# nyu-systems/Grendel-GS

Hardware: NVIDIA B200
Metric: train-step Gaussians/s (preprocess+forward+loss+backward) (higher is better)
Workload: dtype f32

## Files before the change

### grendel-gs_b200/csrc/blend.cu

```cuda
#include "common.cuh"

#define BL_THREADS 256
#define BL_WARPS (BL_THREADS / 32)
#define BL_BLOCKS 16
#ifndef FW_CHUNK
#define FW_CHUNK 256
#endif

#define ALPHA_MIN (1.0f / 255.0f)
#define ALPHA_MAX 0.99f
#define T_EPS 0.0001f
#define FULL 0xffffffffu

GS_D float gs_exp_neg(float x) {
    float y;
    asm("ex2.approx.ftz.f32 %0, %1;" : "=f"(y) : "f"(x * 1.4426950408889634f));
    return y;
}

struct Where { int blk, px, py, half, l16; };
GS_D Where where_am_i(int tile, int gx) {
    Where p;
    const int w = threadIdx.x >> 5, lane = threadIdx.x & 31;
    p.half = lane >> 4;
// ... 174 lines not shown
                        const float test_T = T * (1.f - alpha);
                        if (test_T < T_EPS) {
                            done = true;
                            pxf = qnan;
                            if (STATS) considered = (uint32_t)(base + j + 1);
                        } else {
                            const float2 gb = *reinterpret_cast<const float2 *>(&sr->c);
                            const float w = alpha * T;
                            C0 += b.w * w; C1 += gb.x * w; C2 += gb.y * w;
                            T = test_T;
                            last = (uint32_t)(base + j + 1);
                            if (STATS) blended++;
                        }
                    }
                }
            }
        }
    }
    if (inside) {
        image[pix] = (Ct0 + C0) + T * bg[0];
        image[HW + pix] = (Ct1 + C1) + T * bg[1];
        image[2 * HW + pix] = (Ct2 + C2) + T * bg[2];
        final_T[pix] = T;
        n_contrib[pix] = last;
        if (considered == 0) considered = (uint32_t)total;
    }
    if (CKPT) {
        float r0 = C0, r1 = C1, r2 = C2;
        for (int s = nck - 1; s >= 0; s--) {
            const float4 c = ck[(size_t)s * SEG_SLOT];
            ck[(size_t)s * SEG_SLOT] = make_float4(c.x, r0, r1, r2);
            r0 += c.y; r1 += c.z; r2 += c.w;
        }
        uint32_t m = inside ? last : 0u;
#pragma unroll
        for (int o = 16; o > 0; o >>= 1) m = max(m, __shfl_xor_sync(FULL, m, o));
        if (lane == 0) s_red[threadIdx.x >> 5] = m;
        __syncthreads();
        if (threadIdx.x == 0) {
            uint32_t tl = 0;
#pragma unroll
            for (int w = 0; w < BL_WARPS; w++) tl = max(tl, s_red[w]);
            const uint32_t nseg = (tl + SEG_K - 1) / SEG_K;
            seg.tile_last[blockIdx.x] = tl;
            s_red[BL_WARPS] = nseg;
            s_red[BL_WARPS + 1] = nseg ? atomicAdd(seg.n_units, nseg) : 0u;
        }
        __syncthreads();
        const uint32_t nseg = s_red[BL_WARPS], ubase = s_red[BL_WARPS + 1];
        for (uint32_t i = threadIdx.x; i < nseg; i += BL_THREADS) seg.units[ubase + i] = make_uint2(blockIdx.x, nseg - 1 - i);
    }
    if (STATS) {
        if (threadIdx.x < 3) s_stats[threadIdx.x] = 0ull;
        __syncthreads();
        unsigned long long v0 = inside ? (unsigned long long)total : 0ull, v1 = inside ? considered : 0u,
                           v2 = inside ? blended : 0u;
#pragma unroll
        for (int o = 16; o > 0; o >>= 1) {
            v0 += __shfl_xor_sync(FULL, v0, o);
            v1 += __shfl_xor_sync(FULL, v1, o);
            v2 += __shfl_xor_sync(FULL, v2, o);
        }
        if (lane == 0) { atomicAdd(&s_stats[0], v0); atomicAdd(&s_stats[1], v1); atomicAdd(&s_stats[2], v2); }
        __syncthreads();
        if (threadIdx.x < 3) atomicAdd(&stats[3 * view + threadIdx.x], s_stats[threadIdx.x]);
    }
}

#define F2_THREADS 128
#define F2_WARPS 4
#ifndef F2_MIN_CTAS
#define F2_MIN_CTAS 8
#endif
typedef unsigned long long p2;
GS_D p2 p2_make(float lo, float hi) { p2 r; asm("mov.b64 %0, {%1, %2};" : "=l"(r) : "f"(lo), "f"(hi)); return r; }
GS_D p2 p2_bc(float v) { return p2_make(v, v); }
GS_D float p2_lo(p2 v) { float lo, hi; asm("mov.b64 {%0, %1}, %2;" : "=f"(lo), "=f"(hi) : "l"(v)); return lo; }
GS_D float p2_hi(p2 v) { float lo, hi; asm("mov.b64 {%0, %1}, %2;" : "=f"(lo), "=f"(hi) : "l"(v)); return hi; }
GS_D p2 p2_fma(p2 a, p2 b, p2 c) { p2 r; asm("fma.rn.f32x2 %0, %1, %2, %3;" : "=l"(r) : "l"(a), "l"(b), "l"(c)); return r; }
GS_D p2 p2_mul(p2 a, p2 b) { p2 r; asm("mul.rn.f32x2 %0, %1, %2;" : "=l"(r) : "l"(a), "l"(b)); return r; }
GS_D p2 p2_add(p2 a, p2 b) { p2 r; asm("add.rn.f32x2 %0, %1, %2;" : "=l"(r) : "l"(a), "l"(b)); return r; }
GS_D void p2_fma_acc(p2 &c, p2 a, p2 b) { asm("fma.rn.f32x2 %0, %1, %2, %0;" : "+l"(c) : "l"(a), "l"(b)); }
GS_D void p2_mul_acc(p2 &t, p2 f) { asm("mul.rn.f32x2 %0, %0, %1;" : "+l"(t) : "l"(f)); }

template <bool STATS, bool CKPT>
__global__ void __launch_bounds__(F2_THREADS, F2_MIN_CTAS)
k_blend_fwd2(int W, int H, int tiles_per_view, const float4 *__restrict__ rec, const float *__restrict__ bg,
             const uint8_t *__restrict__ compute_locally, const uint2 *__restrict__ ranges,
             const uint32_t *__restrict__ ids, float *__restrict__ image, float *__restrict__ final_T,
             uint32_t *__restrict__ n_contrib, unsigned long long *__restrict__ stats, const SegWs seg) {
    __shared__ SRec s_rec[FW_CHUNK + 1];
    __shared__ uint16_t s_cull[FW_CHUNK];
    __shared__ unsigned long long s_stats[3];
    __shared__ uint32_t s_red[F2_WARPS + 2];
    const int gx = (W + GS_BLOCK_X - 1) / GS_BLOCK_X;
    const int view = blockIdx.x / tiles_per_view, tile = blockIdx.x - view * tiles_per_view;
    const int warp = threadIdx.x >> 5, lane = threadIdx.x & 31;
    const int quarter = lane >> 3, l8 = lane & 7;
    const int lx = quarter * 4 + (l8 & 1) * 2, ly = warp * 4 + (l8 >> 1);
    const int px = (tile % gx) * GS_BLOCK_X + lx, py = (tile / gx) * GS_BLOCK_Y + ly;
    const bool in0 = px < W && py < H, in1 = px + 1 < W && py < H;
    const size_t HW = (size_t)H * W;
    const size_t pix = (size_t)py * W + px;
    image += (size_t)view * 3 * HW;
    final_T += (size_t)view * HW;
    n_contrib += (size_t)view * HW;
    if (!compute_locally[blockIdx.x]) {
        if (in0) { image[pix] = 0.f; image[HW + pix] = 0.f; image[2 * HW + pix] = 0.f; }
        if (in1) { image[pix + 1] = 0.f; image[HW + pix + 1] = 0.f; image[2 * HW + pix + 1] = 0.f; }
        if (CKPT && threadIdx.x == 0) seg.tile_last[blockIdx.x] = 0u;
        return;
    }
    const uint2 range = ranges[blockIdx.x];
    const int total = (int)(range.y - range.x);
    const float X0 = (float)((tile % gx) * GS_BLOCK_X), Y0 = (float)((tile / gx) * GS_BLOCK_Y);
    const float qnan = __int_as_float(0x7fc00000);
    float npx0 = in0 ? -(float)px : qnan, npx1 = in1 ? -(float)(px + 1) : qnan;
    const float pyf = (float)py;
    const p2 zero2 = p2_bc(0.f), one2 = p2_bc(1.f), mone2 = p2_bc(-1.f);
    p2 T = one2, C0 = zero2, C1 = zero2, C2 = zero2, Ct0 = zero2, Ct1 = zero2, Ct2 = zero2;
    uint32_t last0 = 0, last1 = 0, blended = 0, cons0 = 0, cons1 = 0;
#define F2_DONE (npx0 != npx0 && npx1 != npx1)
    float4 *ck = nullptr;
    int nck = 0;
    if (CKPT)
        ck = seg.ckpt + ((size_t)(range.x / SEG_K) + blockIdx.x) * SEG_SLOT + (warp * 2 + (lx >> 3)) * 32 + (ly & 3) * 8 + (lx & 7);
    for (int i = threadIdx.x; i < FW_CHUNK + 1; i += F2_THREADS) {
        const float4 z = make_float4(0.f, 0.f, 0.f, 0.f);
        s_rec[i].a = z; s_rec[i].b = z; s_rec[i].c = z;
    }
    for (int base = 0; base < total; base += FW_CHUNK) {
        if (__syncthreads_count(F2_DONE) == F2_THREADS) break;
        const int cnt = min(FW_CHUNK, total - base);
        for (int i = threadIdx.x; i < cnt; i += F2_THREADS) {
            const uint32_t g = ids[range.x + base + i];
            const float4 *r = rec + (size_t)3 * g;
            const float4 a = __ldg(r), b = __ldg(r + 1), c = __ldg(r + 2);
            s_rec[i].a = make_float4(a.x, a.y, -a.z, -a.w);
            s_rec[i].b = make_float4(-b.x, b.y, fmaxf(-b.z, 0.f), b.w);
            s_rec[i].c = c;
            const uint16_t m16 = (uint16_t)block_mask16(a, b, c.z, c.w, X0, Y0);
            s_cull[i] = m16;
            if (CKPT) seg.cull[range.x + base + i] = m16;
        }
        __syncthreads();
        for (int g0 = 0; g0 < cnt; g0 += 32) {
            if (__all_sync(FULL, F2_DONE)) break;
            {
                const int e0 = base + g0;
                if (e0 > 0 && (e0 & (SEG_K - 1)) == 0) {
                    if (CKPT) {
                        ck[(size_t)nck * SEG_SLOT] = make_float4(p2_lo(T), p2_lo(C0), p2_lo(C1), p2_lo(C2));
                        ck[(size_t)nck * SEG_SLOT + 1] = make_float4(p2_hi(T), p2_hi(C0), p2_hi(C1), p2_hi(C2));
                        nck++;
                    }
                    Ct0 = p2_add(Ct0, C0); Ct1 = p2_add(Ct1, C1); Ct2 = p2_add(Ct2, C2);
                    C0 = C1 = C2 = zero2;
                }
            }
            const int jj = g0 + 31 - lane;
            const uint32_t m = jj < cnt ? ((uint32_t)s_cull[jj] >> (warp * 4)) : 0u;
            const uint32_t c0 = __ballot_sync(FULL, m & 1u), c1 = __ballot_sync(FULL, m & 2u),
                           c2 = __ballot_sync(FULL, m & 4u), c3 = __ballot_sync(FULL, m & 8u);
            uint32_t mine = quarter == 0 ? c0 : quarter == 1 ? c1 : quarter == 2 ? c2 : c3;
            const p2 npx = p2_make(npx0, npx1);
            p2 npx_cur = npx;
// ... 366 lines not shown
    const uint4 *s_role = &s_role_all[warp][lane];
    const SegCold *s_cold = &s_cold_all[warp];
    const float pxf0 = (float)(X0 + (lane & 7)), pyf0 = (float)(Y0 + (lane >> 3));
    for (int pass = (cnt - 1) / SG_STAGE; pass >= 0; pass--) {
        const int p0 = pass * SG_STAGE;
        __syncwarp();
        const SegCold cold = *s_cold;
        const int pn = min(SG_STAGE, cold.cnt - p0);
        if (lane < pn) {
            const int i = p0 + lane;
            const uint32_t g = cold.ids[i];
            const float4 *r = rec + (size_t)3 * g;
            const float4 a = __ldg(r), b = __ldg(r + 1), c = __ldg(r + 2);
            uint32_t m = cold.cull[i];
            m = (m | (m >> 1)) & 0x5555u;
            m = (m | (m >> 1)) & 0x3333u;
            m = (m | (m >> 2)) & 0x0f0fu;
            m = (m | (m >> 4)) & 0x00ffu;
#pragma unroll
            for (int q = 0; q < 8; q++) {
                const uint32_t bl = ((q < 4 ? cold.blive : cold.blive_hi) >> (8 * (q & 3))) & 0xffu;
                if ((uint32_t)i >= bl) m &= ~(1u << q);
            }
            s_rec[lane].a = make_float4(a.x, a.y, -a.z, -a.w);
            s_rec[lane].b = make_float4(-b.x, b.y, fmaxf(-b.z, 0.f), b.w);
            s_rec[lane].c = make_float4(c.x, c.y, gs_rcp_approx(b.y), __uint_as_float(g));
            s_mask[lane] = m;
        }
        __syncwarp();
        for (int jl = pn - 1; jl >= 0; jl--) {
            const uint32_t m8 = __reduce_or_sync(FULL, s_mask[jl]);
            if (m8 == 0u) continue;
            const int j = p0 + jl;
            const float4 a = s_rec[jl].a, b4 = s_rec[jl].b;
            const float2 c4 = *reinterpret_cast<const float2 *>(&s_rec[jl].c);
            const float mxl = a.x - pxf0, myl = a.y - pyf0;
            float v[9];
#pragma unroll
            for (int q = 0; q < 9; q++) v[q] = 0.f;
            bool any_full = false;
#pragma unroll
            for (int b = 0; b < 8; b++) {
                if (m8 & (1u << b)) {
                    const float4 pc = s_pix[b * 32];
                    const float dx = mxl - (float)((b & 1) * 8), dy = myl - (float)((b >> 1) * 4);
                    const float q = dx * (a.z * dx + a.w * dy) + b4.x * dy * dy;
                    const bool ok = (j < __float_as_int(pc.w)) && __float_as_uint(q) <= __float_as_uint(b4.z);
                    if (__any_sync(FULL, ok)) {
                        const float G = gs_exp_neg(-q);
                        const float alpha = fminf(ALPHA_MAX, b4.y * G);
                        const float ae = ok ? alpha : 0.f;
                        float inv;
                        asm("rcp.approx.ftz.f32 %0, %1;" : "=f"(inv) : "f"(1.f - ae));
                        const float Tk = T[b] * inv;
                        T[b] = Tk;
                        const float cd = b4.w * pc.x + c4.x * pc.y + c4.y * pc.z;
                        const float dL_dalpha = cd * Tk - S[b] * inv;
                        const float mw = ok ? b4.y * dL_dalpha * G : 0.f;
                        const float dch = ae * Tk;
                        S[b] += dch * cd;
                        const float mx_ = mw * dx, my_ = mw * dy;
                        v[0] += mx_; v[1] += my_; v[2] += mx_ * dx; v[3] += mx_ * dy; v[4] += my_ * dy; v[5] += mw;
                        v[6] += dch * pc.x; v[7] += dch * pc.y; v[8] += dch * pc.z;
                        any_full = true;
                    }
                }
            }
            if (!any_full) continue;
            {
                const float sx = v[0], sy = v[1];
                v[0] = 2.f * a.z * sx + a.w * sy;
                v[1] = 2.f * b4.x * sy + a.w * sx;
                v[5] *= s_rec[jl].c.z;
            }
            warp_reduce9(v, lane);
            const uint4 ro = *s_role;
            const float val = (lane == 1 ? v[8] : v[0]) * __uint_as_float(ro.w);
            float *rptr = reinterpret_cast<float *>((unsigned long long)ro.x | ((unsigned long long)ro.y << 32));
            if (rptr) asm volatile("red.global.add.f32 [%0], %1;" ::"l"(rptr + (size_t)__float_as_uint(s_rec[jl].c.w) * ro.z), "f"(val) : "memory");
        }
    }
}

template <bool STATS, bool CKPT>
static void launch_fwd(int grid, cudaStream_t stream, int W, int H, int T1, const float *rec, const float *bg,
                       const uint8_t *cl, const uint32_t *ranges, const uint32_t *ids, float *image, float *final_T,
                       uint32_t *n_contrib, int64_t *stats, const SegWs &seg) {
    if (g_gs_debug_flags & GS_DEBUG_FWD_HALFWARP)
        k_blend_fwd<STATS, CKPT><<<grid, BL_THREADS, 0, stream>>>(
            W, H, T1, reinterpret_cast<const float4 *>(rec), bg, cl, reinterpret_cast<const uint2 *>(ranges), ids, image,
            final_T, n_contrib, reinterpret_cast<unsigned long long *>(stats), seg);
    else
        k_blend_fwd2<STATS, CKPT><<<grid, F2_THREADS, 0, stream>>>(
            W, H, T1, reinterpret_cast<const float4 *>(rec), bg, cl, reinterpret_cast<const uint2 *>(ranges), ids, image,
            final_T, n_contrib, reinterpret_cast<unsigned long long *>(stats), seg);
}

int gs_launch_blend_forward(int num_views, int64_t R, int H, int W, const float *rec, const float *bg,
                            const uint8_t *compute_locally, const uint32_t *ranges, const uint32_t *ids_sorted,
                            float *image, float *final_T, uint32_t *n_contrib, int64_t *stats, void *seg_ws,
                            size_t seg_ws_bytes, cudaStream_t stream) {
    const int gx = (W + GS_BLOCK_X - 1) / GS_BLOCK_X, gy = (H + GS_BLOCK_Y - 1) / GS_BLOCK_Y;
    const int T1 = gx * gy;
    SegWs seg = {nullptr, nullptr, nullptr, nullptr};
    if (seg_ws) {
        if (seg_ws_bytes < seg_bytes(R, (int64_t)T1 * num_views)) {
            gs_set_error("gs_render_forward: segment workspace too small (%zu < %zu)", seg_ws_bytes,
                         seg_bytes(R, (int64_t)T1 * num_views));
            return GS_ENOMEM;
        }
        GS_REQUIRE(((uintptr_t)seg_ws & 255) == 0, "segment workspace must be 256-byte aligned");
        seg = seg_carve(seg_ws, R, (int64_t)T1 * num_views);
        GS_CUDA_TRY(cudaMemsetAsync(seg.n_units, 0, 256, stream));
    }
    if (stats) GS_CUDA_TRY(cudaMemsetAsync(stats, 0, 3 * sizeof(int64_t) * (size_t)num_views, stream));
    GsStageTimer timer(GS_STAGE_BLEND_FWD, stream);
    const int grid = T1 * num_views;
    if (stats && seg_ws)
        launch_fwd<true, true>(grid, stream, W, H, T1, rec, bg, compute_locally, ranges, ids_sorted, image, final_T, n_contrib, stats, seg);
    else if (stats)
        launch_fwd<true, false>(grid, stream, W, H, T1, rec, bg, compute_locally, ranges, ids_sorted, image, final_T, n_contrib, stats, seg);
    else if (seg_ws)
        launch_fwd<false, true>(grid, stream, W, H, T1, rec, bg, compute_locally, ranges, ids_sorted, image, final_T, n_contrib, stats, seg);
    else
        launch_fwd<false, false>(grid, stream, W, H, T1, rec, bg, compute_locally, ranges, ids_sorted, image, final_T, n_contrib, stats, seg);
    GS_LAUNCH_CHECK();
    return GS_OK;
}

extern "C" int gs_render_backward(int P, int64_t R, int image_height, int image_width, const float *rec,
                                  const float *bg, const uint8_t *compute_locally, const uint32_t *ranges,
                                  const uint32_t *ids_sorted, const float *final_T, const uint32_t *n_contrib,
                                  const float *dL_dimage, const void *seg_ws, size_t seg_ws_bytes, float *dL_dmeans2D,
                                  float *dL_dconic_opacity, float *dL_drgb, void *stream) {
    return gs_render_backward_batched(1, P, R, image_height, image_width, rec, bg, compute_locally, ranges, ids_sorted,
                                      final_T, n_contrib, dL_dimage, seg_ws, seg_ws_bytes, dL_dmeans2D, dL_dconic_opacity,
                                      dL_drgb, stream);
}

extern "C" int gs_render_backward_batched(int num_views, int P, int64_t R, int image_height, int image_width,
                                          const float *rec, const float *bg, const uint8_t *compute_locally,
                                          const uint32_t *ranges, const uint32_t *ids_sorted, const float *final_T,
                                          const uint32_t *n_contrib, const float *dL_dimage, const void *seg_ws,
                                          size_t seg_ws_bytes, float *dL_dmeans2D, float *dL_dconic_opacity,
                                          float *dL_drgb, void *stream_) {
    cudaStream_t stream = (cudaStream_t)stream_;
    GS_REQUIRE(num_views >= 1 && num_views <= GS_MAX_VIEWS, "num_views must be in [1, GS_MAX_VIEWS]");
    GS_REQUIRE(P >= 0 && R >= 0 && image_height > 0 && image_width > 0, "sizes");
    if (P == 0) return GS_OK;
    GS_REQUIRE(dL_dmeans2D && dL_dconic_opacity && dL_drgb, "null output");
    if (dL_dmeans2D == dL_dconic_opacity + 4 * (size_t)P && dL_drgb == dL_dmeans2D + 2 * (size_t)P) {
        GS_CUDA_TRY(cudaMemsetAsync(dL_dconic_opacity, 0, sizeof(float) * 9 * (size_t)P, stream));
    } else {
        GS_CUDA_TRY(cudaMemsetAsync(dL_dmeans2D, 0, sizeof(float) * 2 * (size_t)P, stream));
        GS_CUDA_TRY(cudaMemsetAsync(dL_dconic_opacity, 0, sizeof(float) * 4 * (size_t)P, stream));
        GS_CUDA_TRY(cudaMemsetAsync(dL_drgb, 0, sizeof(float) * 3 * (size_t)P, stream));
    }
    if (R == 0) return GS_OK;
    GS_REQUIRE(rec && bg && compute_locally && ranges && ids_sorted && final_T && n_contrib && dL_dimage, "null input");
    const int gx = (image_width + GS_BLOCK_X - 1) / GS_BLOCK_X, gy = (image_height + GS_BLOCK_Y - 1) / GS_BLOCK_Y;
    GsStageTimer timer(GS_STAGE_BLEND_BWD, stream);
    if (seg_ws && !(g_gs_debug_flags & GS_DEBUG_BWD_TILE)) {
        const int64_t T = (int64_t)gx * gy * num_views;
        if (seg_ws_bytes < seg_bytes(R, T)) {
            gs_set_error("gs_render_backward: segment workspace too small");
            return GS_ENOMEM;
        }
        const SegWs seg = seg_carve(const_cast<void *>(seg_ws), R, T);
        const int64_t max_units = R / SEG_K + T;
        k_blend_bwd_seg<<<(unsigned)((max_units + SG_WARPS - 1) / SG_WARPS), SG_THREADS, 0, stream>>>(
            image_width, image_height, gx * gy, reinterpret_cast<const float4 *>(rec), bg,
            reinterpret_cast<const uint2 *>(ranges), ids_sorted, final_T, n_contrib, dL_dimage, seg, dL_dmeans2D,
            dL_dconic_opacity, dL_drgb);
        GS_LAUNCH_CHECK();
        return GS_OK;
    }
    k_blend_bwd<<<gx * gy * num_views, BL_THREADS, 0, stream>>>(
        image_width, image_height, gx * gy, reinterpret_cast<const float4 *>(rec), bg, compute_locally,
        reinterpret_cast<const uint2 *>(ranges), ids_sorted, final_T, n_contrib, dL_dimage, dL_dmeans2D, dL_dconic_opacity,
        dL_drgb);
    GS_LAUNCH_CHECK();
    return GS_OK;
}
```

### grendel-gs_b200/gs_b200/_lib.py

```python
import ctypes as C
import os

_PKG = os.path.dirname(os.path.dirname(os.path.abspath(__file__)))
LIB_PATH = os.environ.get("GS_B200_LIB") or os.path.join(_PKG, "lib", "libgrendel_gs_b200.so")

_vp, _i, _f, _i64, _sz = C.c_void_p, C.c_int, C.c_float, C.c_int64, C.c_size_t

SIGNATURES = {
    "gs_last_error": (C.c_char_p, []),
    "gs_version": (C.c_char_p, []),
    "gs_get_block_xy": (_i, [C.POINTER(_i)] * 3),
    "gs_preprocess_forward": (_i, [_i, _i, _vp, _vp, _f, _vp, _vp, _vp, _vp, _vp, _vp, _i, _i, _f, _f,
                                   _vp, _vp, _vp, _vp, _vp, _vp, _vp]),
    "gs_preprocess_backward": (_i, [_i, _i, _vp, _vp, _f, _vp, _vp, _vp, _vp, _vp, _i, _i, _f, _f, _vp, _vp,
                                    _vp, _vp, _vp, _vp, _vp, _vp, _vp, _vp, _vp]),
    "gs_preprocess_forward_raw": (_i, [_i, _i, _vp, _vp, _vp, _vp, _f, _vp, _vp, _vp, _vp, _vp, _i, _i, _f, _f,
                                       _vp, _vp, _vp, _vp, _vp, _vp, _vp]),
    "gs_preprocess_backward_raw": (_i, [_i, _i, _vp, _vp, _vp, _vp, _f, _vp, _vp, _vp, _vp, _vp, _i, _i, _f, _f,
                                        _vp, _vp, _vp, _vp, _vp, _vp, _vp, _vp, _vp, _vp, _vp, _vp]),
    "gs_preprocess_forward_batched": (_i, [_i, _i, _i, _vp, _vp, _vp, _vp, _f, _vp, _vp, _vp, _i, _i,
                                           _vp, _vp, _vp, _vp, _vp, _vp, _vp]),
    "gs_preprocess_backward_batched": (_i, [_i, _i, _i, _vp, _vp, _vp, _vp, _f, _vp, _vp, _vp, _i, _i, _vp, _vp,
                                            _vp, _vp, _vp, _vp, _vp, _vp, _vp, _vp, _vp, _vp]),
    "gs_get_local2j_ids_bool": (_i, [_i, _i, _i, _i, _vp, _vp, _vp, _vp, _vp]),
# ... 22 lines not shown
    "gs_profile_stage_name": (C.c_char_p, [_i]),
    "gs_debug_set": (_i, [_i]),
    "gs_loss_temp_bytes": (_sz, [_i, _i]),
    "gs_loss_forward": (_i, [_i, _i, _i, _i, _i, _i, _vp, _vp, _vp, _vp, _sz, _vp]),
    "gs_loss_backward": (_i, [_i, _i, _i, _i, _i, _i, _vp, _vp, _vp, _vp, _vp, _vp, _vp]),
    "gs_route_scan_temp_bytes": (_sz, [_i, _i]),
    "gs_route_scan": (_i, [_i, _i, _vp, _vp, _vp, _vp, _sz, _vp]),
    "gs_xchg_temp_bytes": (_sz, [_i, _i, _i]),
    "gs_xchg_route": (_i, [_i, _i, _i, _i, _i, _vp, _vp, _vp, _vp, _vp, _vp, _vp, _vp, _sz, _vp]),
    "gs_xchg_pack": (_i, [_i, _i, _i, _vp, _vp, _vp, _vp, _vp, _vp, _vp, _vp, _vp]),
    "gs_xchg_unpack": (_i, [_i, _vp, _vp, _vp, _vp, _i, _vp, _i, _vp, _vp, _vp, _vp, _vp, _vp]),
    "gs_xchg_pack_grad": (_i, [_i, _vp, _vp, _vp, _vp, _i, _i, _vp, _vp, _vp, _vp, _vp]),
    "gs_xchg_scatter_grad": (_i, [_i, _i, _i, _vp, _vp, _vp, _vp, _vp, _vp, _vp]),
    "gs_adam_step": (_i, [_i, _vp, _vp, _vp, _vp, _vp, _vp, _vp, _vp, _vp, _vp, C.c_float, _vp]),
    "gs_knn3_mean_dist2": (_i, [_i, _vp, _vp, _vp]),
    "gs_densify_temp_bytes": (_sz, [_i]),
    "gs_densify_select": (_i, [_i, _vp, _vp, _vp, _vp, C.c_float, C.c_float, C.c_float, C.c_float, _i, _vp, _sz, _vp, _vp]),
    "gs_densify_gather": (_i, [_i, _i, _i, _i, _vp, _vp, _vp, _vp, _vp, _vp, _vp, _vp, _vp]),
    "gs_peer_alloc": (_i, [_sz, C.POINTER(C.c_void_p), _vp]),
    "gs_peer_open": (_i, [_vp, C.POINTER(C.c_void_p)]),
    "gs_peer_close": (_i, [_vp]),
    "gs_peer_free": (_i, [_vp]),
    "gs_xchg_pack_p2p": (_i, [_i, _i, _i, _vp, _vp, _vp, _vp, _vp, _vp, _vp, _vp, _vp, _vp]),
    "gs_xchg_pack_grad_p2p": (_i, [_i, _vp, _vp, _vp, _vp, _i, _i, _vp, _vp, _vp, _vp, _vp]),
    "gs_xr_temp_bytes": (_sz, [_i, _i, _i]),
    "gs_xr_count": (_i, [_i, _i, _i, _i, _i, _vp, _vp, _vp, _vp, _vp, _vp, _vp, _vp, _sz, _vp]),
    "gs_xr_pack": (_i, [_i, _i, _i, _i, _i, _vp, _vp, _vp, _vp, _vp, _vp, _vp, _vp, _vp, _vp, C.c_longlong, _vp]),
    "gs_xr_pack_dev": (_i, [_i, _i, _i, _i, _i, _vp, _vp, _vp, _vp, _vp, _vp, _vp, _vp, _vp, _vp, _i, _vp, C.c_longlong, _vp]),
    "gs_xr_pull_grad": (_i, [_i, _i, _i, _i, _i, _vp, _vp, _vp, _vp, _vp, _vp, _vp, C.c_longlong, _vp, _vp, _vp, _vp]),
    "gs_sparse_grad_mask": (_i, [_i, _vp, _vp, _vp]),
    "gs_sparse_grad_pack": (_i, [_i, _vp, _vp, _vp, _vp, _vp]),
    "gs_sparse_grad_unpack": (_i, [_i, _vp, _vp, _vp, _vp, _vp]),
    "gs_get_touched_locally": (_i, [_i, _i, _i, _vp, _vp, _vp]),
    "gs_get_pixels_compute_locally_and_in_rect": (_i, [_i, _i, _vp, _i, _i, _i, _i, _vp, _vp]),
    "gs_image_tiles_gather": (_i, [_i, _vp, _vp, _i, _i, _i, _i, _i, _i, _vp, _vp]),
    "gs_image_tiles_scatter_add": (_i, [_i, _vp, _vp, _i, _i, _i, _i, _i, _i, _vp, _vp]),
}


class GsError(RuntimeError):
    pass


_lib = None


def load():
    global _lib
    if _lib is not None:
        return _lib
    if not os.path.exists(LIB_PATH):
        raise ImportError(
            f"{LIB_PATH} is missing: build it with `python -c 'import __graft_entry__ as g; g.build()'` "
            "(nvcc, sm_100a). There is no CPU or PyTorch fallback for this operator.")
    lib = C.CDLL(LIB_PATH)
    for name, (res, args) in SIGNATURES.items():
        fn = getattr(lib, name)
        fn.restype = res
        fn.argtypes = args
    _lib = lib
    return lib


def call(name, *args):
    lib = load()
    rc = getattr(lib, name)(*args)
    if rc != 0:
        raise GsError(f"{name} failed (code {rc}): {lib.gs_last_error().decode(errors='replace')}")


def query(name, *args):
    return getattr(load(), name)(*args)


def ptr(t):
    return None if t is None else t.data_ptr()


STAGE_NUM = 14
DEBUG_NO_BLOCK_CULL = 1
DEBUG_BWD_TILE = 2
DEBUG_FWD_HALFWARP = 4
DEBUG_XR_PACK_CTA = 8


def debug_set(flags):
    return query("gs_debug_set", int(flags))


def profile_enable(on=True):
    call("gs_profile_enable", 1 if on else 0)


def profile_read():
    out = {}
    for st in range(STAGE_NUM):
        ms, n = C.c_double(0.0), C.c_int64(0)
        call("gs_profile_read", st, C.byref(ms), C.byref(n))
        if n.value:
            out[load().gs_profile_stage_name(st).decode()] = (ms.value, n.value)
    return out
```

### include/grendel_gs_b200.h

```cpp
#ifndef GRENDEL_GS_B200_H
#define GRENDEL_GS_B200_H

#include <stddef.h>
#include <stdint.h>

#ifdef __cplusplus
extern "C" {
#endif

#define GS_OK 0
#define GS_EINVAL (-1)
#define GS_ECUDA (-2)
#define GS_ENOMEM (-3)

#define GS_BLOCK_X 16
#define GS_BLOCK_Y 16
#define GS_ONE_DIM_BLOCK_SIZE 256
#define GS_REC_FLOATS 12

#if defined(__GNUC__)
#define GS_API __attribute__((visibility("default")))
#else
#define GS_API
#endif
// ... 48 lines not shown
                                          float *dL_drotation, float *dL_dopacity, void *stream);

GS_API int gs_get_local2j_ids_bool(int P, int image_height, int image_width, int world_size, const float *means2D,
                            const int32_t *radii, const int32_t *strategy, uint8_t *out, void *stream);

GS_API int gs_get_local2j_ids_bool_rects(int P, int image_height, int image_width, int world_size, const float *means2D,
                                  const int32_t *radii, const int32_t *rects, uint8_t *out, void *stream);


GS_API size_t gs_render_count_temp_bytes(int P);

GS_API int gs_render_count(int P, int image_height, int image_width, const float *means2D, const float *conic_opacity,
                           const float *rgb, const float *depths, const int32_t *radii, const uint8_t *compute_locally,
                           uint32_t *order, uint32_t *offsets, float *rec, void *temp, size_t temp_bytes,
                           int64_t *R_host, void *stream);

GS_API size_t gs_render_sort_temp_bytes(int64_t R);

GS_API size_t gs_render_seg_bytes(int64_t R, int num_tiles);

GS_API int gs_render_forward(int P, int64_t R, int image_height, int image_width, const float *means2D,
                             const int32_t *radii, const uint8_t *compute_locally, const uint32_t *order,
                             const uint32_t *offsets, const float *rec, const float *bg, uint32_t *tiles_unsorted,
                             uint32_t *ids_unsorted, uint32_t *tiles_sorted, uint32_t *ids_sorted, void *sort_temp,
                             size_t sort_temp_bytes, uint32_t *ranges, float *image, float *final_T,
                             uint32_t *n_contrib, int64_t *stats, void *seg_ws, size_t seg_ws_bytes, void *stream);

GS_API int gs_render_backward(int P, int64_t R, int image_height, int image_width, const float *rec, const float *bg,
                       const uint8_t *compute_locally, const uint32_t *ranges, const uint32_t *ids_sorted,
                       const float *final_T, const uint32_t *n_contrib, const float *dL_dimage, const void *seg_ws,
                       size_t seg_ws_bytes, float *dL_dmeans2D, float *dL_dconic_opacity, float *dL_drgb, void *stream);

#define GS_MAX_VIEWS 64
GS_API int gs_render_count_batched(int num_views, const int32_t *view_start_host, int image_height, int image_width,
                                   const float *means2D, const float *conic_opacity, const float *rgb,
                                   const float *depths, const int32_t *radii, const uint8_t *compute_locally,
                                   uint32_t *order, uint32_t *offsets, float *rec, void *temp, size_t temp_bytes,
                                   int64_t *R_host, void *stream);
GS_API int gs_render_count_launch(int num_views, const int32_t *view_start_host, int P, int image_height, int image_width,
                                  const float *means2D, const float *conic_opacity, const float *rgb, const float *depths,
                                  const int32_t *radii, const uint8_t *compute_locally, uint32_t *order, uint32_t *offsets,
                                  float *rec, void *temp, size_t temp_bytes, void **ticket, void *stream);
GS_API int gs_render_count_read(void *ticket, int64_t *R_host, void *stream);
GS_API int gs_render_forward_batched(int num_views, const int32_t *view_start_host, int64_t R, int image_height,
                                     int image_width, const float *means2D, const int32_t *radii,
                                     const uint8_t *compute_locally, const uint32_t *order, const uint32_t *offsets,
                                     const float *rec, const float *bg, uint32_t *tiles_unsorted, uint32_t *ids_unsorted,
                                     uint32_t *tiles_sorted, uint32_t *ids_sorted, void *sort_temp,
                                     size_t sort_temp_bytes, uint32_t *ranges, float *image, float *final_T,
                                     uint32_t *n_contrib, int64_t *stats, void *seg_ws, size_t seg_ws_bytes,
                                     void *stream);
GS_API int gs_render_backward_batched(int num_views, int P, int64_t R, int image_height, int image_width,
                                      const float *rec, const float *bg, const uint8_t *compute_locally,
                                      const uint32_t *ranges, const uint32_t *ids_sorted, const float *final_T,
                                      const uint32_t *n_contrib, const float *dL_dimage, const void *seg_ws,
                                      size_t seg_ws_bytes, float *dL_dmeans2D, float *dL_dconic_opacity, float *dL_drgb,
                                      void *stream);

enum {
    GS_STAGE_PREPROCESS_FWD = 0,
    GS_STAGE_COUNT_TILES,
    GS_STAGE_SCAN,
    GS_STAGE_DUPLICATE,
    GS_STAGE_SORT,
    GS_STAGE_RANGES,
    GS_STAGE_BLEND_FWD,
    GS_STAGE_BLEND_BWD,
    GS_STAGE_PREPROCESS_BWD,
    GS_STAGE_LOSS_FWD,
    GS_STAGE_LOSS_BWD,
    GS_STAGE_LOCAL2J,
    GS_STAGE_PACK,
    GS_STAGE_UNPACK,
    GS_STAGE_NUM
};
GS_API int gs_profile_enable(int on);
GS_API int gs_profile_read(int stage, double *total_ms, int64_t *launches);
GS_API const char *gs_profile_stage_name(int stage);

enum {
    GS_DEBUG_NO_BLOCK_CULL = 1,
    GS_DEBUG_BWD_TILE = 2,
    GS_DEBUG_FWD_HALFWARP = 4,
    GS_DEBUG_XR_PACK_CTA = 8
};
GS_API int gs_debug_set(int flags);

GS_API size_t gs_loss_temp_bytes(int rows, int image_width);
GS_API int gs_loss_forward(int image_height, int image_width, int row0, int row1, int count_row0, int count_row1,
                           const float *image, const uint8_t *gt_u8, float *out_l1_ssim, void *temp, size_t temp_bytes,
                           void *stream);
GS_API int gs_loss_backward(int image_height, int image_width, int row0, int row1, int count_row0, int count_row1,
                            const float *image, const uint8_t *gt_u8, const void *temp, const float *grad_l1,
                            const float *grad_ssim, float *dL_dimage, void *stream);

GS_API size_t gs_loss_temp_bytes_batched(int num_views, const int32_t *rows4_host, int image_width);
GS_API int gs_loss_forward_batched(int num_views, int image_height, int image_width, const int32_t *rows4_host,
                                   const float *image, const void *const *gt_u8_ptrs_host, float *out_l1_ssim,
                                   void *temp, size_t temp_bytes, void *stream);
GS_API int gs_loss_backward_batched(int num_views, int image_height, int image_width, const int32_t *rows4_host,
                                    const float *image, const void *const *gt_u8_ptrs_host, const void *temp,
                                    const float *grad_l1, const float *grad_ssim, float *dL_dimage, void *stream);

GS_API size_t gs_route_scan_temp_bytes(int P, int ncols);
GS_API int gs_route_scan(int P, int ncols, const uint8_t *mask, int32_t *gpos, int32_t *colstart, void *temp,
                         size_t temp_bytes, void *stream);

GS_API size_t gs_xchg_temp_bytes(int B, int P, int W);
GS_API int gs_xchg_route(int B, int P, int W, int image_height, int image_width, const void *const *means2D_ptrs_host,
                         const void *const *radii_ptrs_host, const int32_t *row_lo_host, const int32_t *row_hi_host,
                         uint8_t *flags, int32_t *gpos, int32_t *counts, void *temp, size_t temp_bytes, void *stream);
GS_API int gs_xchg_pack(int B, int P, int W, const uint8_t *flags, const int32_t *gpos,
                        const void *const *means2D_ptrs_host, const void *const *rgb_ptrs_host,
                        const void *const *conic_opacity_ptrs_host, const void *const *radii_ptrs_host,
                        const void *const *depths_ptrs_host, float *send_rows, void *stream);
GS_API int gs_xchg_unpack(int nseg, const int32_t *seg_recv_start_host, const int32_t *seg_len_host,
                          const int32_t *seg_cam_host, const int32_t *seg_dst_start_host, int total_rows,
                          const float *recv_rows, int B, void *const *means2D_ptrs_host, void *const *rgb_ptrs_host,
                          void *const *conic_opacity_ptrs_host, void *const *radii_ptrs_host,
                          void *const *depths_ptrs_host, void *stream);
GS_API int gs_xchg_pack_grad(int nseg, const int32_t *seg_recv_start_host, const int32_t *seg_len_host,
                             const int32_t *seg_cam_host, const int32_t *seg_dst_start_host, int total_rows, int B,
                             const void *const *d_means2D_ptrs_host, const void *const *d_rgb_ptrs_host,
                             const void *const *d_conic_opacity_ptrs_host, float *grad_rows, void *stream);
GS_API int gs_xchg_scatter_grad(int B, int P, int W, const uint8_t *flags, const int32_t *gpos, const float *grad_rows,
                                void *const *d_means2D_ptrs_host, void *const *d_rgb_ptrs_host,
                                void *const *d_conic_opacity_ptrs_host, void *stream);

GS_API int gs_peer_alloc(size_t bytes, void **dev_ptr, void *ipc_handle_64);
GS_API int gs_peer_open(const void *ipc_handle_64, void **peer_ptr);
GS_API int gs_peer_close(void *peer_ptr);
GS_API int gs_peer_free(void *dev_ptr);
GS_API int gs_xchg_pack_p2p(int B, int P, int W, const uint8_t *flags, const int32_t *gpos,
                            const void *const *means2D_ptrs_host, const void *const *rgb_ptrs_host,
                            const void *const *conic_opacity_ptrs_host, const void *const *radii_ptrs_host,
                            const void *const *depths_ptrs_host, void *const *dst_rows_ptrs_host,
                            const int32_t *row_delta_host, void *stream);
GS_API int gs_xchg_pack_grad_p2p(int nseg, const int32_t *seg_recv_start_host, const int32_t *seg_len_host,
                                 const int32_t *seg_cam_host, const int32_t *seg_dst_start_host, int total_rows, int B,
                                 const void *const *d_means2D_ptrs_host, const void *const *d_rgb_ptrs_host,
                                 const void *const *d_conic_opacity_ptrs_host, void *const *seg_dst_ptrs_host,
                                 void *stream);

GS_API int gs_xr_pack_dev(int B, int P, int W, int image_height, int image_width, const void *const *means2D_ptrs_host,
                          const void *const *rgb_ptrs_host, const void *const *conic_opacity_ptrs_host,
                          const void *const *radii_ptrs_host, const void *const *depths_ptrs_host,
                          const int32_t *row_lo_host, const int32_t *row_hi_host, const int32_t *blkbase,
                          void *const *peer_recv_ptrs_host, const int32_t *counts_all_dev, int me, int32_t *row0_dev,
                          long long cap_rows, void *stream);
GS_API size_t gs_xr_temp_bytes(int B, int P, int W);
GS_API int gs_xr_count(int B, int P, int W, int image_height, int image_width, const void *const *means2D_ptrs_host,
                       const void *const *radii_ptrs_host, const int32_t *row_lo_host, const int32_t *row_hi_host,
                       int32_t *blkcnt, int32_t *blkbase, int32_t *counts, void *temp, size_t temp_bytes, void *stream);
GS_API int gs_xr_pack(int B, int P, int W, int image_height, int image_width, const void *const *means2D_ptrs_host,
                      const void *const *rgb_ptrs_host, const void *const *conic_opacity_ptrs_host,
                      const void *const *radii_ptrs_host, const void *const *depths_ptrs_host,
                      const int32_t *row_lo_host, const int32_t *row_hi_host, const int32_t *blkbase,
                      void *const *peer_recv_ptrs_host, const int32_t *dst_row0_host, long long cap_rows, void *stream);
GS_API int gs_xr_pull_grad(int B, int P, int W, int image_height, int image_width, const void *const *means2D_ptrs_host,
                           const void *const *radii_ptrs_host, const int32_t *row_lo_host, const int32_t *row_hi_host,
                           const int32_t *blkbase, void *const *peer_grad_ptrs_host, const int32_t *dst_row0_host,
                           long long cap_rows, void *const *d_means2D_ptrs_host, void *const *d_rgb_ptrs_host,
                           void *const *d_conic_opacity_ptrs_host, void *stream);

GS_API int gs_sparse_grad_mask(int P, const float *xyz_grad, uint8_t *mask, void *stream);
GS_API int gs_sparse_grad_pack(int P, const uint8_t *mask, const int32_t *pos, void *const *grads_host, float *rows,
                               void *stream);
// ... 37 lines not shown
```

Before: 729.9 million.

## Add segmented backward blend kernel with compacted staging and paired warp reductions

Adds a new segment-based backward blending kernel that becomes the default, with the old one kept behind a debug flag. It compacts staged Gaussians so that only entries with a non-empty block mask are processed. It accumulates gradients with packed f32x2 arithmetic. It replaces the full 9-value warp reduction per Gaussian with a transpose-style reduce-to-3 and then pairs two Gaussians' reductions before issuing the atomic adds. The goal is fewer shuffle and instruction costs per instance, in exchange for extra shared-memory state and pairing logic.

New measurement: 758.6 million, median of 6. 1.04x the previous value.

```diff
diff --git a/grendel-gs_b200/csrc/blend.cu b/grendel-gs_b200/csrc/blend.cu
--- a/grendel-gs_b200/csrc/blend.cu
+++ b/grendel-gs_b200/csrc/blend.cu
@@ -280,6 +280,7 @@
 GS_D p2 p2_add(p2 a, p2 b) { p2 r; asm("add.rn.f32x2 %0, %1, %2;" : "=l"(r) : "l"(a), "l"(b)); return r; }
 GS_D void p2_fma_acc(p2 &c, p2 a, p2 b) { asm("fma.rn.f32x2 %0, %1, %2, %0;" : "+l"(c) : "l"(a), "l"(b)); }
 GS_D void p2_mul_acc(p2 &t, p2 f) { asm("mul.rn.f32x2 %0, %0, %1;" : "+l"(t) : "l"(f)); }
+GS_D void p2_add_acc(p2 &c, p2 a) { asm("add.rn.f32x2 %0, %0, %1;" : "+l"(c) : "l"(a)); }
 
 template <bool STATS, bool CKPT>
 __global__ void __launch_bounds__(F2_THREADS, F2_MIN_CTAS)
@@ -812,6 +813,237 @@
     }
 }
 
+
+GS_D void warp_reduce9_to3(float v[9], int lane) {
+    {
+        const bool h = lane & 16;
+#pragma unroll
+        for (int i = 0; i < 4; i++) {
+            const float send = h ? v[i] : v[i + 4], keep = h ? v[i + 4] : v[i];
+            v[i] = keep + __shfl_xor_sync(FULL, send, 16);
+        }
+    }
+    {
+        const bool h = lane & 8;
+#pragma unroll
+        for (int i = 0; i < 2; i++) {
+            const float send = h ? v[i] : v[i + 2], keep = h ? v[i + 2] : v[i];
+            v[i] = keep + __shfl_xor_sync(FULL, send, 8);
+        }
+    }
+    v[8] += __shfl_xor_sync(FULL, v[8], 16);
+    v[8] += __shfl_xor_sync(FULL, v[8], 8);
+}
+
+GS_D float warp_reduce_pair(float a0, float a1, float a8, float b0, float b1, float b8, int lane) {
+    const bool h2 = lane & 4, h1 = lane & 2, h0 = lane & 1;
+    const float x = (h2 ? a1 : a0) + __shfl_xor_sync(FULL, h2 ? a0 : a1, 4);
+    const float y = (h2 ? b1 : b0) + __shfl_xor_sync(FULL, h2 ? b0 : b1, 4);
+    float z = (h2 ? b8 : a8) + __shfl_xor_sync(FULL, h2 ? a8 : b8, 4);
+    const float w = (h1 ? y : x) + __shfl_xor_sync(FULL, h1 ? x : y, 2);
+    z += __shfl_xor_sync(FULL, z, 2);
+    return (h0 ? z : w) + __shfl_xor_sync(FULL, h0 ? w : z, 1);
+}
+
+GS_D void seg_red_pair(const uint4 ro, float val, uint32_t id_a, uint32_t id_b, bool only_a) {
+    float *rptr = reinterpret_cast<float *>((unsigned long long)ro.x | ((unsigned long long)ro.y << 32));
+    const bool second = ro.z & 256u;
+    const uint32_t id = second ? id_b : id_a;
+    if (rptr && !(only_a && second))
+        asm volatile("red.global.add.f32 [%0], %1;" ::"l"(rptr + (size_t)id * (ro.z & 255u)), "f"(val * __uint_as_float(ro.w))
+                     : "memory");
+}
+
+struct SegWarp3 {
+    SRec rec[SG_STAGE];
+    float4 pix[8 * 32];
+    uint32_t mask[SG_STAGE];
+    uint4 role[32];
+    float4 pend[32];
+    SegCold cold;
+};
+
+__global__ void __launch_bounds__(SG_THREADS, SG_MIN_CTAS)
+k_blend_bwd_seg3(int W, int H, int tiles_per_view, const float4 *__restrict__ rec, const float *__restrict__ bg,
+                 const uint2 *__restrict__ ranges, const uint32_t *__restrict__ ids, const float *__restrict__ final_T,
+                 const uint32_t *__restrict__ n_contrib, const float *__restrict__ dL_dimage, const SegWs seg,
+                 float *__restrict__ d_means2D, float *__restrict__ d_conic_opacity, float *__restrict__ d_rgb) {
+    __shared__ SegWarp3 s_all[SG_WARPS];
+    const int warp = threadIdx.x >> 5, lane = threadIdx.x & 31;
+    const uint32_t u = blockIdx.x * SG_WARPS + warp;
+    if (u >= *seg.n_units) return;
+    SegWarp3 &sw = s_all[warp];
+    SRec *s_rec = sw.rec;
+    float4 *s_pix = sw.pix + lane;
+    uint32_t *s_mask = sw.mask;
+    const uint2 unit = seg.units[u];
+    const int tile_g = (int)unit.x, sidx = (int)unit.y;
+    const int view = tile_g / tiles_per_view, tile = tile_g - view * tiles_per_view;
+    const int gx = (W + GS_BLOCK_X - 1) / GS_BLOCK_X;
+    const uint2 range = ranges[tile_g];
+    const int tl = (int)seg.tile_last[tile_g];
+    const int seg_base = sidx * SEG_K;
+    const int cnt = min(SEG_K, tl - seg_base);
+    const size_t HW = (size_t)H * W;
+    final_T += (size_t)view * HW;
+    n_contrib += (size_t)view * HW;
+    dL_dimage += (size_t)view * 3 * HW;
+    const int X0 = (tile % gx) * GS_BLOCK_X, Y0 = (tile / gx) * GS_BLOCK_Y;
+    const float bg0 = bg[0], bg1 = bg[1], bg2 = bg[2];
+    const float4 *ck = seg.ckpt + ((size_t)(range.x / SEG_K) + tile_g + sidx) * SEG_SLOT + lane;
+    float T[8], S[8];
+    uint32_t blive = 0, blive_hi = 0;
+#pragma unroll
+    for (int b = 0; b < 8; b++) {
+        const int px = X0 + (b & 1) * 8 + (lane & 7), py = Y0 + (b >> 1) * 4 + (lane >> 3);
+        const bool inside = px < W && py < H;
+        const size_t pix = (size_t)py * W + px;
+        float Tf = 0.f, d0 = 0.f, d1 = 0.f, d2 = 0.f;
+        int last = 0;
+        if (inside) {
+            Tf = final_T[pix];
+            last = (int)n_contrib[pix];
+            d0 = dL_dimage[pix]; d1 = dL_dimage[HW + pix]; d2 = dL_dimage[2 * HW + pix];
+        }
+        const float sbg = Tf * (bg0 * d0 + bg1 * d1 + bg2 * d2);
+        T[b] = Tf;
+        S[b] = sbg;
+        if (last > seg_base + SEG_K) {
+            const float4 c = ck[b * 32];
+            T[b] = c.x;
+            S[b] = c.y * d0 + c.z * d1 + c.w * d2 + sbg;
+        }
+        const int live = max(0, min(SEG_K, last - seg_base));
+        s_pix[b * 32] = make_float4(d0, d1, d2, __int_as_float(live));
+        const uint32_t m = __reduce_max_sync(FULL, (uint32_t)live);
+        if (b < 4) blive |= m << (8 * b); else blive_hi |= m << (8 * (b - 4));
+    }
+    {
+        const bool even = !(lane & 1);
+        const int role = even ? (lane >> 2) : (lane == 1 || lane == 5 ? 8 : -1);
+        const uint32_t second = even ? (lane >> 1) & 1 : (lane >> 2) & 1;
+        float *rptr = nullptr;
+        uint32_t rstride = 0;
+        float rscale = 0.f;
+        if (role >= 0) {
+            if (role < 2) { rptr = d_means2D + role; rstride = 2; rscale = role == 0 ? -0.5f * (float)W : -0.5f * (float)H; }
+            else if (role < 6) { rptr = d_conic_opacity + (role - 2); rstride = 4; rscale = role == 3 ? -1.f : (role == 5 ? 1.f : -0.5f); }
+            else { rptr = d_rgb + (role - 6); rstride = 3; rscale = 1.f; }
+        }
+        const unsigned long long rp = (unsigned long long)rptr;
+        sw.role[lane] = make_uint4((uint32_t)rp, (uint32_t)(rp >> 32), rstride | (second << 8), __float_as_uint(rscale));
+        if (lane == 0) {
+            SegCold c;
+            c.ids = ids + range.x + seg_base; c.cull = seg.cull + range.x + seg_base; c.cnt = cnt; c.blive = blive; c.blive_hi = blive_hi;
+            sw.cold = c;
+        }
+    }
+    const uint4 *s_role = &sw.role[lane];
+    const SegCold *s_cold = &sw.cold;
+    const float pxf0 = (float)(X0 + (lane & 7)), pyf0 = (float)(Y0 + (lane >> 3));
+    float4 *s_pend = &sw.pend[lane];
+    bool pend = false;
+    for (int p0 = (cnt - 1) & ~(SG_STAGE - 1); p0 >= 0; p0 -= SG_STAGE) {
+        __syncwarp();
+        const SegCold cold = *s_cold;
+        const int pn = min(SG_STAGE, cold.cnt - p0);
+        uint32_t m = 0u;
+        if (lane < pn) {
+            const int i = p0 + lane;
+            m = cold.cull[i];
+            m = (m | (m >> 1)) & 0x5555u;
+            m = (m | (m >> 1)) & 0x3333u;
+            m = (m | (m >> 2)) & 0x0f0fu;
+            m = (m | (m >> 4)) & 0x00ffu;
+#pragma unroll
+            for (int q = 0; q < 8; q++) {
+                const uint32_t bl = ((q < 4 ? cold.blive : cold.blive_hi) >> (8 * (q & 3))) & 0xffu;
+                if ((uint32_t)i >= bl) m &= ~(1u << q);
+            }
+        }
+        const uint32_t act = __ballot_sync(FULL, m != 0u);
+        if (m != 0u) {
+            const int slot = __popc(act & ((1u << lane) - 1u));
+            const uint32_t g = cold.ids[p0 + lane];
+            const float4 *r = rec + (size_t)3 * g;
+            const float4 a = __ldg(r), b = __ldg(r + 1), c = __ldg(r + 2);
+            s_rec[slot].a = make_float4(a.x, a.y, -a.z, -a.w);
+            s_rec[slot].b = make_float4(-b.x, b.y, fmaxf(-b.z, 0.f), b.w);
+            s_rec[slot].c = make_float4(c.x, c.y, gs_rcp_approx(b.y), __uint_as_float(g));
+            s_mask[slot] = m | ((uint32_t)lane << 8);
+        }
+        __syncwarp();
+        for (int k = __popc(act) - 1; k >= 0; k--) {
+            const uint32_t mw8 = __reduce_or_sync(FULL, s_mask[k]);
+            const uint32_t m8 = mw8 & 0xffu;
+            const int j = p0 + (int)(mw8 >> 8);
+            const float4 a = s_rec[k].a, b4 = s_rec[k].b;
+            const float2 c4 = *reinterpret_cast<const float2 *>(&s_rec[k].c);
+            const float mxl = a.x - pxf0, myl = a.y - pyf0;
+            const p2 zero2 = p2_bc(0.f);
+            p2 s01 = zero2, s23 = zero2, s67 = zero2;
+            float s4 = 0.f, s5 = 0.f, s8 = 0.f;
+            bool any_full = false;
+#pragma unroll
+            for (int b = 0; b < 8; b++) {
+                if (m8 & (1u << b)) {
+                    const float4 pc = s_pix[b * 32];
+                    const float dx = mxl - (float)((b & 1) * 8), dy = myl - (float)((b >> 1) * 4);
+                    const float q = dx * (a.z * dx + a.w * dy) + b4.x * dy * dy;
+                    const bool ok = (j < __float_as_int(pc.w)) && __float_as_uint(q) <= __float_as_uint(b4.z);
+                    if (__any_sync(FULL, ok)) {
+                        const float G = gs_exp_neg(-q);
+                        const float alpha = fminf(ALPHA_MAX, b4.y * G);
+                        const float ae = ok ? alpha : 0.f;
+                        float inv;
+                        asm("rcp.approx.ftz.f32 %0, %1;" : "=f"(inv) : "f"(1.f - ae));
+                        const float Tk = T[b] * inv;
+                        T[b] = Tk;
+                        const float cd = b4.w * pc.x + c4.x * pc.y + c4.y * pc.z;
+                        const float dL_dalpha = cd * Tk - S[b] * inv;
+                        const float mw = ok ? b4.y * dL_dalpha * G : 0.f;
+                        const float dch = ae * Tk;
+                        S[b] += dch * cd;
+                        const p2 d = p2_make(dx, dy);
+                        const p2 mxy = p2_mul(p2_bc(mw), d);
+                        p2_add_acc(s01, mxy);
+                        p2_fma_acc(s23, p2_bc(p2_lo(mxy)), d);
+                        s4 += p2_hi(mxy) * dy;
+                        s5 += mw;
+                        p2_fma_acc(s67, p2_bc(dch), p2_make(pc.x, pc.y));
+                        s8 += dch * pc.z;
+                        any_full = true;
+                    }
+                }
+            }
+            if (!any_full) continue;
+            float v[9];
+            {
+                const float sx = p2_lo(s01), sy = p2_hi(s01);
+                v[0] = 2.f * a.z * sx + a.w * sy;
+                v[1] = 2.f * b4.x * sy + a.w * sx;
+                v[2] = p2_lo(s23); v[3] = p2_hi(s23); v[4] = s4;
+                v[5] = s5 * s_rec[k].c.z;
+                v[6] = p2_lo(s67); v[7] = p2_hi(s67); v[8] = s8;
+            }
+            warp_reduce9_to3(v, lane);
+            const uint32_t id = __float_as_uint(s_rec[k].c.w);
+            if (!pend) {
+                *s_pend = make_float4(v[0], v[1], v[8], __uint_as_float(id));
+                pend = true;
+                continue;
+            }
+            const float4 pa = *s_pend;
+            seg_red_pair(*s_role, warp_reduce_pair(pa.x, pa.y, pa.z, v[0], v[1], v[8], lane), __float_as_uint(pa.w), id, false);
+            pend = false;
+        }
+    }
+    if (pend) {
+        const float4 pa = *s_pend;
+        seg_red_pair(*s_role, warp_reduce_pair(pa.x, pa.y, pa.z, 0.f, 0.f, 0.f, lane), __float_as_uint(pa.w), 0u, true);
+    }
+}
+
 template <bool STATS, bool CKPT>
 static void launch_fwd(int grid, cudaStream_t stream, int W, int H, int T1, const float *rec, const float *bg,
                        const uint8_t *cl, const uint32_t *ranges, const uint32_t *ids, float *image, float *final_T,
@@ -898,10 +1130,17 @@
         }
         const SegWs seg = seg_carve(const_cast<void *>(seg_ws), R, T);
         const int64_t max_units = R / SEG_K + T;
-        k_blend_bwd_seg<<<(unsigned)((max_units + SG_WARPS - 1) / SG_WARPS), SG_THREADS, 0, stream>>>(
-            image_width, image_height, gx * gy, reinterpret_cast<const float4 *>(rec), bg,
-            reinterpret_cast<const uint2 *>(ranges), ids_sorted, final_T, n_contrib, dL_dimage, seg, dL_dmeans2D,
-            dL_dconic_opacity, dL_drgb);
+        const unsigned grid = (unsigned)((max_units + SG_WARPS - 1) / SG_WARPS);
+        if (g_gs_debug_flags & GS_DEBUG_BWD_SEG_R2)
+            k_blend_bwd_seg<<<grid, SG_THREADS, 0, stream>>>(
+                image_width, image_height, gx * gy, reinterpret_cast<const float4 *>(rec), bg,
+                reinterpret_cast<const uint2 *>(ranges), ids_sorted, final_T, n_contrib, dL_dimage, seg, dL_dmeans2D,
+                dL_dconic_opacity, dL_drgb);
+        else
+            k_blend_bwd_seg3<<<grid, SG_THREADS, 0, stream>>>(
+                image_width, image_height, gx * gy, reinterpret_cast<const float4 *>(rec), bg,
+                reinterpret_cast<const uint2 *>(ranges), ids_sorted, final_T, n_contrib, dL_dimage, seg, dL_dmeans2D,
+                dL_dconic_opacity, dL_drgb);
         GS_LAUNCH_CHECK();
         return GS_OK;
     }
diff --git a/grendel-gs_b200/gs_b200/_lib.py b/grendel-gs_b200/gs_b200/_lib.py
--- a/grendel-gs_b200/gs_b200/_lib.py
+++ b/grendel-gs_b200/gs_b200/_lib.py
@@ -128,6 +128,7 @@
 DEBUG_BWD_TILE = 2
 DEBUG_FWD_HALFWARP = 4
 DEBUG_XR_PACK_CTA = 8
+DEBUG_BWD_SEG_R2 = 16
 
 
 def debug_set(flags):
diff --git a/include/grendel_gs_b200.h b/include/grendel_gs_b200.h
--- a/include/grendel_gs_b200.h
+++ b/include/grendel_gs_b200.h
@@ -154,7 +154,8 @@
     GS_DEBUG_NO_BLOCK_CULL = 1,
     GS_DEBUG_BWD_TILE = 2,
     GS_DEBUG_FWD_HALFWARP = 4,
-    GS_DEBUG_XR_PACK_CTA = 8
+    GS_DEBUG_XR_PACK_CTA = 8,
+    GS_DEBUG_BWD_SEG_R2 = 16
 };
 GS_API int gs_debug_set(int flags);
 
diff --git a/profiles/predict_seg3.py b/profiles/predict_seg3.py
--- /dev/null
+++ b/profiles/predict_seg3.py
@@ -0,0 +1,94 @@
+import os
+import sys
+
+import numpy as np
+
+ROOT = os.path.dirname(os.path.dirname(os.path.abspath(__file__)))
+sys.path[:0] = [ROOT, os.path.join(ROOT, "grendel-gs_b200"), os.path.join(ROOT, "tests")]
+from gs_b200 import synthetic as syn
+from oracle.oracle import Oracle
+from test_band_cull import ellipse_bands, make_records
+
+F = np.float32
+SEG_K = 32 * 4
+COST = {
+    "r2": dict(unit=120, pass_=40, empty=13, head=34, bit=2, block=11, body=31, tail=70, pair_extra=0),
+    "r3": dict(unit=130, pass_=55, empty=0, head=27, bit=2, block=11, body=29, tail=45, pair_extra=46),
+}
+
+
+def main():
+    W, H, n = 480, 270, 125_000
+    cam = syn.make_camera(W, H)
+    sc = syn.make_scene(n, W, H, seed=0)
+    o = Oracle(np.float32, threads=max(1, (os.cpu_count() or 8) // 2))
+    pre = o.preprocess_forward(sc["means3D"], sc["scales"], sc["rotations"], sc["shs"], sc["opacities"], cam)
+    gx, gy = (W + 15) // 16, (H + 15) // 16
+    fwd = o.render_forward(H, W, pre["means2D"], pre["conic_opacity"], pre["rgb"], pre["depths"], pre["radii"],
+                           np.ones(gx * gy, np.uint8), (0, 0, 0))
+    rec = make_records(pre["means2D"], pre["conic_opacity"])
+    ids, ranges = fwd["ids"].astype(np.int64), fwd["ranges"].reshape(-1, 2)
+    R = int(fwd["R"])
+    yy, xx = np.meshgrid(np.arange(16), np.arange(16), indexing="ij")
+    lx, ly = xx.reshape(-1), yy.reshape(-1)
+    blk_of_pix = (ly // 4) * 2 + lx // 8
+    ev = dict(units=0, passes=0, staged=0, empty=0, nonempty=0, blocks=0, passed=0, tails=0, pairs=0)
+    for tile in range(gx * gy):
+        beg, end = ranges[tile]
+        X0, Y0 = (tile % gx) * 16, (tile // gx) * 16
+        px, py = X0 + lx, Y0 + ly
+        inside = (px < W) & (py < H)
+        last = np.where(inside, fwd["n_contrib"][np.minimum(py, H - 1), np.minimum(px, W - 1)], 0).astype(np.int64)
+        tl = int(last.max())
+        if end <= beg or tl == 0:
+            continue
+        g = ids[beg:end][:tl]
+        bands = ellipse_bands(rec, g, X0, Y0)
+        mask = np.zeros((8, tl), bool)
+        for q in range(4):
+            bl, bh = bands[q]
+            for half in range(2):
+                mask[2 * q + half] = (bh >= 8 * half) & (bl <= 8 * half + 7)
+        dx = rec["mx"][g][None, :] - px[:, None].astype(F)
+        dy = rec["my"][g][None, :] - py[:, None].astype(F)
+        power = dx * (rec["az"][g] * dx + rec["aw"][g] * dy) + rec["bx"][g] * dy * dy
+        passes_px = (power >= rec["thr"][g]) & (power <= 0) & (np.arange(tl)[None, :] < last[:, None])
+        for s in range((tl + SEG_K - 1) // SEG_K):
+            sb = s * SEG_K
+            cnt = min(SEG_K, tl - sb)
+            live = np.clip(last - sb, 0, SEG_K)
+            ev["units"] += 1
+            ev["passes"] += (cnt + 31) // 32
+            pend = False
+            for i in range(cnt):
+                e = sb + i
+                m = np.array([mask[b, e] and i < live[blk_of_pix == b].max() for b in range(8)])
+                ev["staged"] += 1
+                if not m.any():
+                    ev["empty"] += 1
+                    continue
+                ev["nonempty"] += 1
+                ev["blocks"] += int(m.sum())
+                full = False
+                for b in np.nonzero(m)[0]:
+                    if passes_px[blk_of_pix == b, e].any():
+                        ev["passed"] += 1
+                        full = True
+                if full:
+                    ev["tails"] += 1
+                    ev["pairs"] += int(pend)
+                    pend = not pend
+    print(f"scene: {n} Gaussians @ {W}x{H}: R = {R} instances")
+    print("events: " + ", ".join(f"{k} {v}" for k, v in ev.items()))
+    print(f"staged entries with an empty trimmed mask: {ev['empty'] / ev['staged']:.3f} of {ev['staged']}")
+    print(f"per instance: blocks in the mask {ev['blocks'] / R:.2f}, blocks past the vote {ev['passed'] / R:.2f}, "
+          f"reduction tails {ev['tails'] / R:.2f}")
+    for name, c in COST.items():
+        tot = (c["unit"] * ev["units"] + c["pass_"] * ev["passes"] + c["empty"] * ev["empty"] +
+               (c["head"] + 7 * c["bit"]) * ev["nonempty"] + c["block"] * ev["blocks"] + c["body"] * ev["passed"] +
+               c["tail"] * ev["tails"] + c["pair_extra"] * ev["pairs"])
+        print(f"{name}: {tot:.3e} warp instructions (x16 for c2: {16 * tot:.3e}), {tot / R:.1f} per instance")
+
+
+if __name__ == "__main__":
+    main()
diff --git a/profiles/r3_compare_outputs.py b/profiles/r3_compare_outputs.py
--- /dev/null
+++ b/profiles/r3_compare_outputs.py
@@ -0,0 +1,31 @@
+import os
+import sys
+
+import numpy as np
+
+
+def main(old_a, old_b, new):
+    names = sorted(f[:-4] for f in os.listdir(old_a) if f.endswith(".npy"))
+    ok = True
+    for k in names:
+        a, b, n = (np.load(os.path.join(d, k + ".npy")).astype(np.float64) for d in (old_a, old_b, new))
+        if k in ("loss", "sample_rows", "radii"):
+            same = np.array_equal(a, n) and np.array_equal(a, b)
+            ok &= same
+            print(f"{k:22s} bit-identical: {same}" + (f"   ({float(a):.9f})" if k == "loss" else ""))
+            continue
+        d_oo, d_no = np.abs(a - b), np.abs(n - a)
+        r_oo, r_no = float(np.sqrt((d_oo ** 2).mean())), float(np.sqrt((d_no ** 2).mean()))
+        m_oo, m_no = float(d_oo.max()), float(d_no.max())
+        scale = float(np.sqrt((a ** 2).mean()))
+        good = m_no <= 2 * m_oo and r_no <= 2 * r_oo
+        ok &= good
+        print(f"{k:22s} rms {scale:.3e}   old-vs-old max {m_oo:.3e} rms {r_oo:.3e}   new-vs-old max {m_no:.3e} "
+              f"rms {r_no:.3e}   ratio max {m_no / max(m_oo, 1e-300):.2f} rms {r_no / max(r_oo, 1e-300):.2f}   "
+              f"{'ok' if good else 'FAIL'}")
+    print("all within 2x the run-to-run difference" if ok else "FAILED")
+    return 0 if ok else 1
+
+
+if __name__ == "__main__":
+    sys.exit(main(*sys.argv[1:4]))
```
